# OpenMatchmaking/microservice-matchmaking

Hardware: AMD Instinct MI355X
Metric: matched players/sec over 1M-player pool (higher is better)
Workload: dtype int32

## Files before the change

### microservice_matchmaking_amd/csrc/mm_engine.hip

```cpp
#include <hip/hip_runtime.h>

#include <stdint.h>
#include <stdio.h>
#include <stdlib.h>
#include <string.h>
#include <time.h>

#include <dlfcn.h>

#include <algorithm>
#include <mutex>
#include <cmath>
#include <new>
#include <vector>

#include "../../include/mm_engine.h"
#include "../../include/mm_wait.h"
#include <mm_gfx950.h>


#define MM_NO_SLOT 0xFFFFFFFFu
#define MM_ST_FREE 0
#define MM_ST_LIVE 1
#define MM_ST_CANCELLED 2
// ... 774 lines not shown
    for (uint32_t k = 0; k < A.L; ++k) dst[k] = src[k];
    pk[(size_t)A.total * A.L + i] = __float_as_uint(out_score[(size_t)g * A.out_rec_stride + j]);
    pk[(size_t)A.total * (A.L + 1u) + i] = out_pass[(size_t)g * A.out_rec_stride + j];
}
__global__ __launch_bounds__(256) void k_wait_matched(PackArgs A, const uint32_t* __restrict__ out_slots,
                                                      const uint32_t* __restrict__ stamp, uint32_t capacity, uint32_t now,
                                                      uint32_t* __restrict__ wait)
{
    const uint32_t i = blockIdx.x * blockDim.x + threadIdx.x;
    if (i >= A.total * A.L) return;
    const uint32_t lobby = i / A.L;
    uint32_t g = 0;
    while (g + 1u < A.n_groups && lobby >= A.pre[g + 1u]) ++g;
    const uint32_t sl = out_slots[(size_t)g * A.out_slot_stride + (size_t)(i - A.pre[g] * A.L)];
    wait[i] = sl < capacity ? now - stamp[sl] : 0u;
}
#define MM_PACK_MAX 8192u

struct TailArgs {
    uint32_t pre[MM_MAX_GROUPS + 1];
    uint32_t from[MM_MAX_GROUPS], base[MM_MAX_GROUPS];
    uint32_t n_groups, L, total, out_slot_stride, out_rec_stride;
};
__global__ __launch_bounds__(256) void k_results_tail(TailArgs A, const uint32_t* __restrict__ out_slots,
                                                      const float* __restrict__ out_score, const uint32_t* __restrict__ out_pass,
                                                      uint32_t* __restrict__ h_slots, float* __restrict__ h_score, uint32_t* __restrict__ h_pass)
{
    const uint32_t i = blockIdx.x * blockDim.x + threadIdx.x;
    if (i >= A.total) return;
    uint32_t g = 0;
    while (g + 1u < A.n_groups && i >= A.pre[g + 1u]) ++g;
    const uint32_t j = A.from[g] + (i - A.pre[g]);
    const size_t at = (size_t)A.base[g] + j;
    const uint32_t* const src = out_slots + (size_t)g * A.out_slot_stride + (size_t)j * A.L;
    for (uint32_t k = 0; k < A.L; ++k) h_slots[at * A.L + k] = src[k];
    h_score[at] = out_score[(size_t)g * A.out_rec_stride + j];
    h_pass[at] = out_pass[(size_t)g * A.out_rec_stride + j];
}
#define MM_TAIL_MAX (1u << 20)

__global__ __launch_bounds__(256) void k_look(const uint32_t* __restrict__ src, uint32_t* __restrict__ dst_host, uint32_t nwords,
                                              uint32_t* seq_host, uint32_t seq)
{
    for (uint32_t i = threadIdx.x; i < nwords; i += blockDim.x) dst_host[i] = src[i];
    __threadfence_system();
    __syncthreads();
    if (threadIdx.x == 0) __hip_atomic_store(seq_host, seq, __ATOMIC_RELEASE, __HIP_MEMORY_SCOPE_SYSTEM);
}

#include "mm_pair.inc"
#include "mm_team.inc"

static __device__ __forceinline__ bool pair_chain_is_fast(const struct PairChain* pc, uint32_t g)
{
    return pc[g].fast != 0u;
// ... 76 lines not shown
    uint32_t* d_tk_chunkB;
    uint32_t* d_tk_fdone;
    uint32_t team_seq;
    uint32_t* d_tk_sqi;
    uint32_t tk_memb;
    uint32_t tk_chunk_stride;
    std::vector<uint32_t> tk_last_len;
    uint32_t dbg_last_w, dbg_last_c;
    ChainDev* h_chains;
    uint32_t* h_counters;
    std::vector<uint8_t> h_state;
    uint32_t next_slot;
    uint32_t cancel_pending;
    std::vector<uint32_t> r_released;
    uint32_t* h_rslots;
    float* h_rscore;
    uint32_t* h_rpass;
    uint32_t r_n, r_L;
    hipStream_t copy_stream;
    hipEvent_t ev_copy;
    bool ev_copy_pending;
    uint32_t r_base[MM_MAX_GROUPS], r_cnt[MM_MAX_GROUPS], r_pre[MM_MAX_GROUPS + 1];
    uint32_t r_sent[MM_MAX_GROUPS];
    uint32_t r_marked[MM_MAX_GROUPS];
    bool r_based;
    bool poisoned;
    uint32_t ticks_seen;
    bool clock_on;
    uint32_t clock_now;
    uint32_t* d_stamp;
    uint32_t* d_wt_rows;
    uint32_t wt_max_chunks;
    uint32_t* d_wt_out;
    WaitGroupDev* d_wt_stats;
    uint32_t* d_wt_matched;
    std::vector<uint32_t> x_slot, x_group, x_age;
    std::vector<uint32_t> x_new;
    std::vector<int32_t> x_rating;
    std::vector<uint32_t> x_cons, x_stamp;
    uint32_t* d_mv_cols;
    uint8_t* d_mv_group;
    uint32_t* h_mwait;
    uint32_t mw_n;
    uint32_t* d_loc_tag;
    uint32_t* d_loc_rows;
    uint32_t loc_max_chunks;
// ... 772 lines not shown
        if (live.empty()) return MM_OK;
        MMTRY(ensure_staging(e, live.size()));
        const uint32_t k = (uint32_t)live.size();
        HIPCHK(e, hipMemcpyAsync(e->d_in_slot, live.data(), k * sizeof(uint32_t), hipMemcpyHostToDevice, e->stream));
        hipLaunchKernelGGL(k_cancel, dim3((k + 255) / 256), dim3(256), 0, e->stream, k, e->d_in_slot, e->d_state);
        HIPCHK(e, hipGetLastError());
        HIPCHK(e, hipStreamSynchronize(e->stream));
        e->cancel_pending += k;
        return MM_OK;
    });
}

#ifndef MM_RESULTS_MIN_PAIR
#define MM_RESULTS_MIN_PAIR 16384u
#endif
#ifndef MM_RESULTS_MIN_TEAM
#define MM_RESULTS_MIN_TEAM 4096u
#endif
static void results_set_bases(mm_engine* e, const uint32_t* before, uint32_t L)
{
    uint32_t run = 0;
    for (uint32_t g = 0; g < e->cfg.n_groups; ++g) {
        e->r_base[g] = run;
        run += before[g] / L + 1u;
    }
    e->r_based = true;
}

static void results_mark(mm_engine* e, uint32_t g, uint32_t to, uint32_t L)
{
    const uint32_t from = e->r_marked[g];
    if (to <= from) return;
    const uint32_t* const sl = e->h_rslots + (size_t)(e->r_base[g] + from) * L;
    for (size_t i = 0, n = (size_t)(to - from) * L; i < n; ++i) e->h_state[sl[i]] = MM_ST_FREE;
    e->r_marked[g] = to;
}

static int results_absorb(mm_engine* e, uint32_t L)
{
    if (!e->ev_copy_pending) return MM_OK;
    HIPCHK(e, hipEventSynchronize(e->ev_copy));
    e->ev_copy_pending = false;
    for (uint32_t g = 0; g < e->cfg.n_groups; ++g) results_mark(e, g, e->r_sent[g], L);
    return MM_OK;
}

static int results_send(mm_engine* e, const uint32_t* n_out, uint32_t L, uint32_t min_new, bool* on_main = nullptr)
{
    uint32_t fresh = 0;
    for (uint32_t g = 0; g < e->cfg.n_groups; ++g) fresh += n_out[g] > e->r_sent[g] ? n_out[g] - e->r_sent[g] : 0u;
    if (on_main) *on_main = false;
    if (fresh < min_new) return MM_OK;
    MMTRY(results_absorb(e, L));
    if (on_main != nullptr && fresh <= MM_TAIL_MAX && e->tn.results_tail) {
        TailArgs A;
        memset(&A, 0, sizeof(A));
        A.n_groups = e->cfg.n_groups; A.L = L; A.out_slot_stride = e->out_slot_stride; A.out_rec_stride = e->out_rec_stride;
        for (uint32_t g = 0; g < e->cfg.n_groups; ++g) {
            const uint32_t a = e->r_sent[g], b = n_out[g] > a ? n_out[g] : a;
            A.from[g] = a; A.base[g] = e->r_base[g]; A.pre[g + 1u] = A.pre[g] + (b - a);
            e->r_sent[g] = b;
        }
        A.total = A.pre[e->cfg.n_groups];
        if (A.total) {
            hipLaunchKernelGGL(k_results_tail, dim3((A.total + 255u) / 256u), dim3(256), 0, e->stream, A, e->d_out_slots, e->d_out_score,
                               e->d_out_pass, e->h_rslots, e->h_rscore, e->h_rpass);
            HIPCHK(e, hipGetLastError());
        }
        *on_main = true;
        return MM_OK;
    }
    const bool main_st = on_main != nullptr && fresh <= 8192u;
    hipStream_t const st = main_st ? e->stream : e->copy_stream;
    for (uint32_t g = 0; g < e->cfg.n_groups; ++g) {
        const uint32_t a = e->r_sent[g], b = n_out[g];
        if (b <= a) continue;
        const size_t at = (size_t)e->r_base[g] + a;
        HIPCHK(e, hipMemcpyAsync(&e->h_rslots[at * L], e->d_out_slots + (size_t)g * e->out_slot_stride + (size_t)a * L,
                                 (size_t)(b - a) * L * sizeof(uint32_t), hipMemcpyDeviceToHost, st));
        HIPCHK(e, hipMemcpyAsync(&e->h_rscore[at], e->d_out_score + (size_t)g * e->out_rec_stride + a, (size_t)(b - a) * sizeof(float),
                                 hipMemcpyDeviceToHost, st));
        HIPCHK(e, hipMemcpyAsync(&e->h_rpass[at], e->d_out_pass + (size_t)g * e->out_rec_stride + a, (size_t)(b - a) * sizeof(uint32_t),
                                 hipMemcpyDeviceToHost, st));
        e->r_sent[g] = b;
    }
    if (main_st) { *on_main = true; return MM_OK; }
    HIPCHK(e, hipEventRecord(e->ev_copy, e->copy_stream));
    e->ev_copy_pending = true;
    return MM_OK;
// ... 148 lines not shown
    {
        uint32_t seg = 256u, stage = NXI_STAGE;
        while (seg < NXI_SEG && (unsigned long long)bound > 8192ull * seg) seg <<= 1;
        if (e->tn.pair_nxseg) seg = e->tn.pair_nxseg;
        if (e->tn.pair_nxstage) stage = e->tn.pair_nxstage;
        if (stage < seg + 64u) stage = seg + 64u;
        if (stage > NXI_STAGE) stage = NXI_STAGE;
        const bool timing = (cfg.flags & MM_CFG_TIMING) != 0;
        if (timing) HIPCHK(e, hipEventRecord(e->ev_nx[0], e->stream));
        hipLaunchKernelGGL(kp_nx_init, dim3((bound + seg - 1u) / seg + 1u, G), dim3(NXI_THREADS), 0, e->stream, P, seg, stage);
        if (timing) { HIPCHK(e, hipEventRecord(e->ev_nx[1], e->stream)); e->ev_nx_set = true; }
    }
    HIPCHK(e, hipGetLastError());
    uint32_t tail_no[MM_MAX_GROUPS];
    bool tail_send = false;
    memset(e->ps_hand, 0, sizeof(e->ps_hand));
    if (bound >= PL_MAX) {
        uint32_t tiles = (bound + PK_T - 1u) / PK_T + 1u;
        if (tiles > e->pk_max_tiles) tiles = e->pk_max_tiles;
        bool after_persist = false;
        uint32_t last_tp = 0;
        uint32_t idle_looks = 0;
        unsigned long long last_progress = ~0ull;
        for (uint32_t guard = 0;; ++guard) {
            if (idle_looks > 64u) return MM_ERR_INTERNAL;
            MMTRY(look_launch(e, e->d_pchains, e->h_pchains, G * sizeof(PairChain)));
            MMTRY(look_wait(e));
            ++e->ps.host_looks;
            if (e->tn.debug && guard >= 200u && guard % 200u == 0u) {
                fprintf(stderr, "[mm-pair] look %u: cool-down %u, persist %d, last tile length %u;", guard, e->pair_pcool, (int)kp_rounds_on(e), last_tp);
                for (uint32_t g = 0; g < G; ++g) {
                    const PairChain& pc = e->h_pchains[g];
                    if (pc.fast) fprintf(stderr, " g%u[stage %u m %u qlen %u passes %u compact %u pfail 0x%x]", g, pc.stage, pc.m, pc.qlen, pc.passes, pc.want_compact, pc.pfail);
                }
                fprintf(stderr, "\n");
            }
            {
                unsigned long long progress = 0;
                for (uint32_t g = 0; g < G; ++g) {
                    const PairChain& pc = e->h_pchains[g];
                    if (pc.fast) progress += (unsigned long long)pc.passes + ((unsigned long long)pc.m << 32) + (pc.stage == PS_TILED ? 1u : 0u) + pc.want_compact;
                }
                idle_looks = progress == last_progress ? idle_looks + 1u : 0u;
                last_progress = progress;
            }
            bool tiled = false, compact = false;
// ... 25 lines not shown
                uint32_t bf[MM_MAX_GROUPS];
                for (uint32_t g = 0; g < G; ++g) { bf[g] = e->h_pchains[g].before; sent_no[g] = e->h_pchains[g].fast ? e->h_pchains[g].n_out : 0u; }
                if (!e->r_based) results_set_bases(e, bf, M.L);
            }
            after_persist = false;
            for (uint32_t g = 0; g < G; ++g) {
                const PairChain& pc = e->h_pchains[g];
                if (!pc.fast) continue;
                if (pc.ppass > e->ps.pair_rounds_passes) e->ps.pair_rounds_passes = pc.ppass;
                if (pc.rounds > e->ps.pair_tiled_passes) e->ps.pair_tiled_passes = pc.rounds;
            }
            for (uint32_t g = 0; g < G; ++g) {
                const PairChain& pc = e->h_pchains[g];
                e->ps_hand[0][g] = pc.fast ? pc.passes : 0u;
                e->ps_hand[1][g] = pc.fast ? pc.n_out : 0u;
                e->ps_hand[2][g] = pc.fast ? pc.ppass : 0u;
                e->ps_hand[3][g] = pc.fast ? pc.ptm[15] : 0u;
            }
            if (!tiled) {
                if (guard) { for (uint32_t g = 0; g < G; ++g) tail_no[g] = sent_no[g]; tail_send = true; }
                break;
            }
            bool want_fit = false;
            uint32_t yield_q = 0, yield_g = 0;
            if (kp_rounds_on(e) && !e->pair_pcool && !compact && !e->tn.pair_tile_fixed) {
                uint32_t gl = 0;
                for (uint32_t g = 1; g < G; ++g)
                    if (P.bm[g] > P.bm[gl]) gl = g;
                const PairChain& pc = e->h_pchains[gl];
                if (P.bm[gl]) {
                    uint32_t capq = e->tn.pair_ptiles * PK_TMAX;
                    for (uint32_t tlen = PK_TMAX; tlen >= PK_TMAX / 4u && pc.m <= e->tn.pair_ptiles * tlen; tlen >>= 1) capq = e->tn.pair_ptiles * (tlen >> 1);
                    if (pc.m <= e->tn.pair_ptiles * (PK_TMAX / 4u)) capq = PL_MAX - 1u;
                    if (pc.qlen <= capq && pc.m > capq && capq >= PL_MAX) {
                        hipLaunchKernelGGL(kp_ask_compact, dim3(G), dim3(64), 0, e->stream, P, 1u << gl);
                        compact = true;
                    } else {
                        if (pc.m > e->tn.pair_ptiles * PK_TMAX) want_fit = true;
                        yield_q = capq;
                        yield_g = gl;
                    }
                }
            }
            uint32_t tp = PK_TMAX;
            bool persist = kp_rounds_on(e) && !compact && (longest + PK_TMAX - 1u) / PK_TMAX <= e->tn.pair_ptiles;
            if (persist && e->pair_pcool) { --e->pair_pcool; persist = false; e->ps.degraded = 1; }
            if (!kp_rounds_on(e) && !compact && (longest + PK_TMAX - 1u) / PK_TMAX <= e->tn.pair_ptiles) e->ps.degraded = 1;
            const uint32_t cap_p = e->tn.pair_ptiles < e->tn.pair_tiles_max ? e->tn.pair_ptiles : e->tn.pair_tiles_max;
            const uint32_t tiles_max = kp_rounds_on(e) ? cap_p : e->tn.pair_tiles_max;
            if (!e->tn.pair_tile_fixed)
                for (uint32_t cand = PK_TMAX / 4u; cand < PK_TMAX; cand <<= 1)
                    if ((longest + cand - 1u) / cand <= tiles_max) { tp = cand; break; }
            if (last_tp && tp > last_tp && !compact) {
                hipLaunchKernelGGL(kp_ask_compact, dim3(G), dim3(64), 0, e->stream, P, 0xFFFFFFFFu);
                compact = true;
                last_tp = 0;
            }
            tiles = (longest + tp - 1u) / tp;
#define TILE_LAUNCH(KERNEL, GRID, BLOCK, ...)                                                                              \
    do {                                                                                                                   \
        if (tp == PK_TMAX) hipLaunchKernelGGL(KERNEL<PK_TMAX>, GRID, BLOCK, 0, e->stream, __VA_ARGS__);                    \
// ... 27 lines not shown
                    if (slots) {
                        P.grp = 0;
                        const uint32_t K = e->tn.pair_pbatch, slice = MM_PERSIST_SLICE ? MM_PERSIST_SLICE : K + 1u;
                        for (uint32_t it = 0; it <= K; it += slice)
                            TILE_LAUNCH(kp_rounds, dim3(8u * slots), dim3(PT_THREADS), P, it, it + slice < K + 1u ? it + slice : K + 1u, K);
                        ++e->ps.pair_rounds_launches;
                        after_persist = true;
                        COMPACT_LAUNCH();
                        HIPCHK(e, hipGetLastError());
                        MMTRY(results_absorb(e, M.L));
                        MMTRY(results_send(e, sent_no, M.L, e->tn.results_early ? MM_RESULTS_MIN_PAIR : 0xFFFFFFFFu));
                        continue;
                    }
                    P.xslots = 0;
                }
                if (e->tn.pair_xcd) {
                    const uint32_t slots = pair_xcd_map(P, tof, G);
                    if (slots) rgrid = dim3(8u * slots);
                }
                uint32_t r = e->round_ctr;
                TILE_LAUNCH(kp_round, rgrid, dim3(PT_THREADS), P, r, 1u);
                ++r;
                if (P.grp) TILE_LAUNCH(kp_group, dim3(ngr, G), dim3(1024), P, r);
                for (uint32_t b = 0; b < (want_fit && e->tn.pair_batch > 12u ? 12u : e->tn.pair_batch); ++b) {
                    TILE_LAUNCH(kp_round, rgrid, dim3(PT_THREADS), P, r, 0u);
                    ++e->ps.pair_round_launches;
                    ++r;
                    if (P.grp) TILE_LAUNCH(kp_group, dim3(ngr, G), dim3(1024), P, r);
                }
                TILE_LAUNCH(kp_round_commit, dim3(tiles, G), dim3(256), P, r);
                hipLaunchKernelGGL(kp_round_stage, dim3(G), dim3(64), 0, e->stream, P, r);
                COMPACT_LAUNCH();
                e->round_ctr = r;
            }
#undef COMPACT_LAUNCH
#undef TILE_LAUNCH
            HIPCHK(e, hipGetLastError());
            MMTRY(results_absorb(e, M.L));
            MMTRY(results_send(e, sent_no, M.L, e->tn.results_early ? MM_RESULTS_MIN_PAIR : 0xFFFFFFFFu));
        }
    }
    hipLaunchKernelGGL(kp_late, dim3(G), dim3(PL_THREADS), 0, e->stream, P);
    hipLaunchKernelGGL(kp_finish, dim3(G), dim3(1024), 0, e->stream, P);
    HIPCHK(e, hipGetLastError());
    if (tail_send) {
        MMTRY(results_absorb(e, M.L));
        MMTRY(results_send(e, tail_no, M.L, e->tn.results_early ? MM_RESULTS_MIN_PAIR : 0xFFFFFFFFu));
// ... 411 lines not shown
    const bool use_pair = M.team_size == 1u && M.teams == 2u && !e->tn.force_generic;
    if (use_pair) {
        RoctxRange rr("mm_tick/pair walk");
        e->ps.paths |= MM_PATH_PAIR;
        MMTRY(pair_walk(e, mode, M, purge));
    }
    bool team_any = false;
    if (!use_pair && !e->tn.force_generic && e->live_upper >= TT_MIN) {
        RoctxRange rr("mm_tick/team walk");
        MMTRY(team_walk(e, mode, M, purge, &team_any));
        if (team_any) e->ps.paths |= MM_PATH_TEAM;
    }
    if (!e->ps.paths) e->ps.paths = MM_PATH_GENERIC;
    WalkParams P;
    walk_params_common(P, e, mode, purge);
    P.out_cap = (cfg.capacity + MM_MAX_LOBBY) / M.L + 1u;
    P.max_passes = 0x7FFFFFFFu;
    P.M = M;
    P.pskip = use_pair ? e->d_pchains : NULL;
    P.tskip = team_any ? e->d_tchains : NULL;
    hipLaunchKernelGGL(k_walk, dim3(G), dim3(WK_THREADS), 0, e->stream, P);
    HIPCHK(e, hipGetLastError());
    if (timing) HIPCHK(e, hipEventRecord(e->ev[2], e->stream));
    HIPCHK(e, hipMemcpyAsync(e->h_chains, e->d_chains, e->n_chains * sizeof(ChainDev), hipMemcpyDeviceToHost, e->stream));
    HIPCHK(e, hipMemcpyAsync(e->h_counters, e->d_counters, sizeof(uint32_t), hipMemcpyDeviceToHost, e->stream));
    if (use_pair) HIPCHK(e, hipMemcpyAsync(e->h_pchains, e->d_pchains, G * sizeof(PairChain), hipMemcpyDeviceToHost, e->stream));
    HIPCHK(e, hipStreamSynchronize(e->stream));
    const double t_copy0 = host_now_ms();
    if (use_pair && e->tn.debug) MMTRY(report_pair(e));

    uint32_t total = 0, after = 0, before = 0, pmax = 0, errf = 0;
    unsigned long long pairs = 0, scanned = 0;
    for (uint32_t g = 0; g < G; ++g) {
        const ChainDev& c = e->h_chains[mode * G + g];
        total += c.n_out;
        after += c.len + c.lobby.n;
        before += c.before;
        pairs += c.pairs;
        scanned += c.scanned;
        errf |= c.err;
        if (c.passes > pmax) pmax = c.passes;
    }
    if (errf) return MM_ERR_INTERNAL;
    if (e->tn.fail_tick && ++e->ticks_seen == e->tn.fail_tick) return MM_ERR_INTERNAL;
    if ((size_t)total * M.L > (size_t)cfg.capacity + (size_t)MM_MAX_LOBBY * G) return MM_ERR_INTERNAL;
    RoctxRange rr_res("mm_tick/match list");
    bool tail_on_main = false;
    {
        uint32_t bf[MM_MAX_GROUPS], no[MM_MAX_GROUPS];
        for (uint32_t g = 0; g < G; ++g) {
            const ChainDev& c = e->h_chains[mode * G + g];
            bf[g] = c.n_out * M.L;
            no[g] = c.n_out;
            if (e->r_based && (c.n_out < e->r_sent[g] || (unsigned long long)c.n_out * M.L > (unsigned long long)c.before + M.L))
                return MM_ERR_INTERNAL;
        }
        if (!e->r_based && total > 0u && total <= MM_PACK_MAX) {
            const PackArgs A = pack_args(e, mode, M.L, total);
            for (uint32_t g = 0; g < G; ++g) { e->r_base[g] = A.pre[g]; e->r_sent[g] = no[g]; }
            e->r_based = true;
            hipLaunchKernelGGL(k_pack_results, dim3((total + 255u) / 256u), dim3(256), 0, e->stream, A, e->d_out_slots, e->d_out_score,
                               e->d_out_pass, e->d_pack);
            HIPCHK(e, hipGetLastError());
            HIPCHK(e, hipMemcpyAsync(e->h_rslots, e->d_pack, (size_t)total * M.L * sizeof(uint32_t), hipMemcpyDeviceToHost, e->stream));
            HIPCHK(e, hipMemcpyAsync(e->h_rscore, e->d_pack + (size_t)total * M.L, (size_t)total * sizeof(float), hipMemcpyDeviceToHost, e->stream));
            HIPCHK(e, hipMemcpyAsync(e->h_rpass, e->d_pack + (size_t)total * (M.L + 1u), (size_t)total * sizeof(uint32_t), hipMemcpyDeviceToHost, e->stream));
            tail_on_main = true;
        } else {
            if (!e->r_based) results_set_bases(e, bf, M.L);
            MMTRY(results_send(e, no, M.L, 1u, &tail_on_main));
        }
    }
    const uint32_t nrel = e->h_counters[0];
    e->r_released.resize(nrel);
    if (nrel)
        HIPCHK(e, hipMemcpyAsync(e->r_released.data(), e->d_released, nrel * sizeof(uint32_t), hipMemcpyDeviceToHost, e->stream));
    if (e->clock_on && total > 0u) {
        const PackArgs A = pack_args(e, mode, M.L, total);
        const uint32_t words = total * M.L;
        hipLaunchKernelGGL(k_wait_matched, dim3((words + 255u) / 256u), dim3(256), 0, e->stream, A, e->d_out_slots, e->d_stamp,
                           cfg.capacity, e->clock_now, e->d_wt_matched);
        HIPCHK(e, hipGetLastError());
        HIPCHK(e, hipMemcpyAsync(e->h_mwait, e->d_wt_matched, (size_t)words * sizeof(uint32_t), hipMemcpyDeviceToHost, e->stream));
    }
    {
        MMTRY(results_absorb(e, M.L));
    }
    e->r_pre[0] = 0;
    for (uint32_t g = 0; g < G; ++g) {
        e->tk_last_len[mode * G + g] = e->h_chains[mode * G + g].len + e->h_chains[mode * G + g].lobby.n;
        e->r_cnt[g] = e->h_chains[mode * G + g].n_out;
        e->r_pre[g + 1u] = e->r_pre[g] + e->r_cnt[g];
    }
    HIPCHK(e, hipStreamSynchronize(e->stream));
    if (tail_on_main)
        for (uint32_t g = 0; g < G; ++g) results_mark(e, g, e->r_sent[g], M.L);
    for (uint32_t i = 0; i < nrel; ++i) e->h_state[e->r_released[i]] = MM_ST_FREE;
    e->cancel_pending = e->cancel_pending >= nrel ? e->cancel_pending - nrel : 0;
    {
        const unsigned long long gone = (unsigned long long)total * M.L + nrel;
        e->live_upper = e->live_upper >= gone ? e->live_upper - gone : 0;
    }
    e->r_n = total;
    e->mw_n = e->clock_on ? total : 0u;
    if (n_matches) *n_matches = total;
    if (e->ps.paths & MM_PATH_PAIR) path_stats_pair(e, mode);
    e->ps.crit_team_group = 0xFFFFFFFFu;
    if (e->ps.paths & MM_PATH_TEAM) path_stats_team(e);
    if (stats) {
        memset(stats, 0, sizeof(*stats));
        stats->pool_before = before;
        stats->pool_after = after;
        stats->matches = total;
        stats->players_matched = total * M.L;
        stats->passes_max = pmax;
        stats->chains = G;
        stats->pairs = pairs;
// ... 954 lines not shown
```

### microservice_matchmaking_amd/csrc/mm_pair.inc

```

#define PK_NO 0xFFFFFFFFu
#define PK_ABORT 0xFFFFFFFEu

#define NX_INV 0u
#define NX_NONE 0xFFFFu
#define NX_FAR 0xFFFEu

#ifndef PK_T
#define PK_T 8192u
#endif
enum : uint32_t { PK_TMAX = PK_T };
#undef PK_T
static constexpr uint32_t PK_T = PK_TMAX;
#ifndef PK_TILES_MAX
#define PK_TILES_MAX 40u
#endif
#define PK_XSEG 4u
#ifndef PK_GS
#define PK_GS 8u
#endif
#ifndef PK_GROUP_MIN
#define PK_GROUP_MIN 64u
#endif
#ifndef PL_MAX
// ... 1793 lines not shown
#undef EMIT_STORE
#undef SEAT_PATCH
}

#define PF_TIMEOUT 1u
#define PF_XCD 2u
#define PF_INJECT 3u
#define PF_YIELD 4u

template <uint32_t TP>
struct RoundsRes {
    alignas(16) uint32_t key[2 * TP + 64];
    alignas(16) uint16_t nx[TP];
    alignas(16) uint16_t g[TP + 8];
    alignas(16) uint32_t pc[TP + 64];
    alignas(16) uint32_t bits[2 * TP / 32 + 4];
    uint32_t cnt[16];
    uint16_t nw[TP / 32 + 2];
    uint16_t path[TP / 2 + 72];
    RoundState S, N;
    uint32_t my[8];
    uint32_t ctl[4];
    uint32_t tm[16];
};

static __device__ __forceinline__ uint32_t w_scan_fit_x(const uint32_t* key, const uint32_t* bits, uint32_t akey, uint32_t from, uint32_t m,
                                                        uint32_t w, int lane)
{
    uint32_t klo, krng;
    pk_bounds(akey, w, klo, krng);
    for (uint32_t p = from; p < m; p += 256u) {
        uint32_t bw[4], kv[4];
#pragma unroll
        for (uint32_t u = 0; u < 4u; ++u) {
            const uint32_t c = p + 64u * u + (uint32_t)lane;
            bw[u] = c < m ? xld(bits + (c >> 5)) : 0u;
            kv[u] = c < m ? key[c] : 0xFFFFFFFFu;
        }
#pragma unroll
        for (uint32_t u = 0; u < 4u; ++u) {
            const uint32_t c = p + 64u * u + (uint32_t)lane;
            const unsigned long long b = __ballot(((bw[u] >> (c & 31u)) & 1u) != 0u && pk_in(kv[u], klo, krng));
            if (b) return p + 64u * u + (uint32_t)__ffsll(b) - 1u;
        }
    }
    return PK_NO;
// ... 29 lines not shown
                t = ((sg >> 8) & 0xFFu) + sl * (sg >> 16);
                found = true;
            }
            if (!found) sl -= c;
        }
        if (!found) return;
    }
    PairChain* const pc = P.pchains + g;
    const uint32_t m = P.bm[g], buf = P.bbuf[g];
    if (m == 0u || t >= (m + PK_T - 1u) / PK_T) return;
    const int tid_o = threadIdx.x;
    const uint32_t w = P.window, ntiles = (m + PK_T - 1u) / PK_T;
    const uint32_t c = P.mode * P.n_groups + g;
    const size_t qo = (size_t)c * P.capacity, po = (size_t)g * P.pstride;
    const uint32_t base = t * PK_T;
    const uint32_t tl = dev_min_u32(PK_T, m - base);
    const uint32_t hl = dev_min_u32(2u * PK_T, m - base);
    const uint32_t* const key = P.key[buf] + po;
    const uint32_t* const oidx = P.oidx[buf] + po;
    uint16_t* const gnx = P.nx16[buf] + po + base;
    uint32_t* const bits_com = P.bits[buf] + (size_t)g * P.bits_stride;
    const uint32_t own_words = (tl + 31u) >> 5, hwords = (hl + 31u) >> 5;
    unsigned long long* const bar = P.pbar + g;
    long long tq = clock64();
#define TMARK(K_) do { if (tmr) { const long long now = clock64(); L.tm[K_] += (uint32_t)(now - tq); tq = now; } } while (0)

    if (it_begin == 0u) {
        const int tid = tid_o;
        MM_RESIDENT_FRESH(L);
        if (tid == 0) {
            RoundState S;
            S.live = 1; S.done = 0; S.want_compact = 0; S.rounds = pc->rounds;
            S.qlen = pc->qlen; S.passes = pc->passes; S.n_out = pc->n_out; S.has_anchor = pc->has_anchor;
            S.a_key = pc->a_key; S.a_slot = pc->a_slot; S.a_cons = pc->a_cons; S.a_team = pc->a_team;
            S.a_rating = pc->a_rating; S.pairs = pc->pairs; S.scanned = pc->scanned;
            S.pos0 = pc->pos0; S.changed0 = pc->changed0; S.extra0 = pc->extra0; S.a_oi = PK_NO;
            L.S = S;
            L.N = S;
            L.ctl[0] = 0; L.ctl[1] = 0; L.ctl[2] = 0;
            for (int k = 0; k < 16; ++k) L.tm[k] = 0;
        }
        for (uint32_t i = tid; i < 2u * PK_T / 32u + 4u; i += PT_THREADS) s_bits[i] = i < hwords ? bits_com[(base >> 5) + i] : 0u;
        copy_words_x4((uint32_t*)s_nx, (const uint32_t*)gnx, (tl + 1u) >> 1, tid, PT_THREADS);
        if (tid < 8) s_g[PK_T + tid] = (uint16_t)PK_T;
        if (tid == 0) { s_cnt[1] = 0; s_cnt[2] = 0; s_cnt[3] = 0; s_cnt[4] = 0; }
        if ((uint32_t)tid < RP_MAXLONG) s_pc[RP_MAXLONG + tid] = PK_NO;
        __syncthreads();
        prep_stage_keys<PK_T>(s_key, s_bits, key + base, hl, tid);
        __syncthreads();
    } else if (L.ctl[0]) return;

    uint32_t stop = 0;
    bool ended = false;
    uint32_t tst = 0;
    long long dw0 = 0;
    uint32_t dwork = 0, dn = 0;
    for (uint32_t it = it_begin; it < it_end; ++it) {
        int tid_l = tid_o;
        TW_LAUNDER(tid_l);
        const int tid = tid_l, lane = tid & 63, wave = tid >> 6;
        const bool tmr = t == 1u && tid == 0;
        const uint32_t cpar = it & 1u, npar = cpar ^ 1u;
        const uint32_t* const bits_src = P.bitsp[cpar] + (size_t)g * P.bits_stride;
        uint32_t* const bits_dst = P.bitsp[npar] + (size_t)g * P.bits_stride;
        uint32_t em_off = PK_NO, em_ia = 0, em_iq = 0, em_score = 0, hd_off = PK_NO, hd_iq = 0, hd_score = 0;
        uint32_t em_sa = 0, em_sq = 0, hd_sq = 0, hd_sa = 0, hd_team = 0, em_pass = 0;
        bool em_loaded = false;
#define EMIT_LOAD() do { if (!em_loaded) { em_loaded = true;                                                   \
        if (em_off != PK_NO) { em_sa = P.q_slot[qo + em_ia]; em_sq = P.q_slot[qo + em_iq]; }                  \
        if (hd_off != PK_NO) hd_sq = P.q_slot[qo + hd_iq]; } } while (0)
#define EMIT_STORE() do { EMIT_LOAD();                                                                         \
        uint32_t* const eos = P.out_slots + (size_t)g * P.out_slot_stride;                                    \
        if (em_off != PK_NO) {                                                                                \
            eos[2u * em_off] = em_sa; eos[2u * em_off + 1u] = em_sq;                                          \
            P.out_score[(size_t)g * P.out_rec_stride + em_off] = (float)(int32_t)em_score;                    \
            P.out_pass[(size_t)g * P.out_rec_stride + em_off] = em_pass; }                                    \
        if (hd_off != PK_NO) {                                                                                \
            eos[2u * hd_off + hd_team] = hd_sa; eos[2u * hd_off + (1u - hd_team)] = hd_sq;                    \
            P.out_score[(size_t)g * P.out_rec_stride + hd_off] = (float)(int32_t)hd_score;                    \
            P.out_pass[(size_t)g * P.out_rec_stride + hd_off] = em_pass; }                                    \
        em_off = PK_NO; hd_off = PK_NO; } while (0)

        if (it > 0u) {
            if (tid == 0) {
// ... 8 lines not shown
                    if ((wv & 0xFFFFFFFFull) >= need) break;
                    if (f == 0u && xld(P.pyield) != 0u) {
                        const unsigned long long nv = wv | ((unsigned long long)(PF_YIELD | (it << 8)) << 32);
                        if (atomicCAS(bar, wv, nv) == wv) { verdict = PF_YIELD | (it << 8); break; }
                        continue;
                    }
                    if (f == 0u && wall_clock64() - t0 > limit) {
                        const unsigned long long nv = wv | ((unsigned long long)(PF_TIMEOUT | (it << 8)) << 32);
                        if (atomicCAS(bar, wv, nv) == wv) { verdict = PF_TIMEOUT | (it << 8); break; }
                        continue;
                    }
                    __builtin_amdgcn_s_sleep(1);
                }
                if (!verdict && it == 1u) {
                    const uint32_t xm = xld(P.pxmask + g);
                    if (xm & (xm - 1u)) verdict = PF_XCD | (1u << 8);
                }
                L.ctl[1] = verdict;
            }
            __syncthreads();
            tw_sinv();
            if (L.ctl[1]) { stop = L.ctl[1]; break; }
            TMARK(0);
            if (tid == 0 && (P.tune & 0x10000u)) dw0 = clock64();
            const RoundState S = L.S;
            em_pass = S.passes;
            if (wave != 0) {
                for (uint32_t i = PK_T / 32u + (uint32_t)tid - 64u; i < hwords; i += PT_THREADS - 64u) {
                    const uint32_t nw_ = xld(bits_src + (base >> 5) + i);
                    uint32_t gone = s_bits[i] & ~nw_;
                    s_bits[i] = nw_;
                    while (gone) {
                        const uint32_t b = (uint32_t)__ffs((int)gone) - 1u;
                        gone &= gone - 1u;
                        s_key[(i << 5) + b] |= PK_DEAD;
                    }
                }
                if ((uint32_t)tid - 64u < RP_MAXLONG) s_pc[RP_MAXLONG + tid - 64] = PK_NO;
                __builtin_amdgcn_fence(__ATOMIC_RELEASE, "workgroup");
                wave_lockstep();
                if (lane == 0) atomicAdd(&s_cnt[4], 1u);
                while (lds_ld(&s_cnt[4]) < (uint32_t)(PT_THREADS / 64 - 1)) __builtin_amdgcn_s_sleep(1);
                __builtin_amdgcn_fence(__ATOMIC_ACQUIRE, "workgroup");
                if (it != K && !(P.tune & 0x4000u))
                    repair_sweep<PK_T>(s_key, s_nx, s_pc, &s_cnt[1], s_pc + 2u * RP_MAXLONG + (uint32_t)wave * RP_TODO, bits_src + (base >> 5),
                                       tl, hl, base + hl == m, w, lane, (uint32_t)wave - 1u, PT_THREADS / 64u - 1u, tst);
            }
// ... 196 lines not shown
                        em_score = sc;
                    } else {
                        os[2u * (my_off + i)] = P.q_slot[qo + oidx[base + a]];
                        os[2u * (my_off + i) + 1u] = P.q_slot[qo + oidx[qabs]];
                        P.out_score[(size_t)g * P.out_rec_stride + my_off + i] = (float)(int32_t)sc;
                        P.out_pass[(size_t)g * P.out_rec_stride + my_off + i] = em_pass;
                    }
                }
            }
            if (tid == 0) {
                if (n) {
                    const uint32_t a = s_path[n - 1u], o = s_nx[a];
                    const bool internal = o != NX_NONE && o != NX_FAR && a + o < tl;
                    if (internal && d != DISP_NONE) atomicOr(&pc->err, MM_ERRF_SEAT_INVARIANT);
                } else if (d != DISP_NONE) atomicOr(&pc->err, MM_ERRF_SEAT_INVARIANT);
                L.S = L.N;
                L.ctl[2] += 1u;
            }
            __syncthreads();
            TMARK(9);
        }
        struct { uint32_t live, has_anchor, a_key; } N;
        N.live = L.S.live; N.has_anchor = L.S.has_anchor; N.a_key = L.S.a_key;
        if (!N.live || it == K) { EMIT_STORE(); ended = true; break; }
        if (it > 0u && L.S.qlen <= P.pyq[g]) {
            if (t == 0u && tid == 0) __hip_atomic_store(P.pyield, 1u, __ATOMIC_RELAXED, __HIP_MEMORY_SCOPE_AGENT);
            EMIT_STORE(); ended = true; break;
        }

        for (uint32_t i = tid; i < own_words; i += PT_THREADS) bits_dst[(base >> 5) + i] = s_bits[i];
        if (tid == 0) { s_cnt[0] = PK_NO; s_cnt[4] = 0; }
        prep_repair<PK_T>(s_key, s_nx, s_pc, &s_cnt[1], bits_src + (base >> 5), tl, hl, base + hl == m, w, tid, tst,
                          tmr ? L.tm : nullptr);
        EMIT_LOAD();
        if (N.has_anchor) {
            uint32_t klo, krng;
            pk_bounds(N.a_key, w, klo, krng);
            uint32_t best = PK_NO;
            for (uint32_t i = tid; i < tl; i += PT_THREADS)
                if (best == PK_NO && pk_in(s_key[i], klo, krng)) best = i;
            const unsigned long long b = __ballot(best != PK_NO);
            if (b) {
                uint32_t v = best;
                for (int dd = 1; dd < 64; dd <<= 1) { const uint32_t o2 = (uint32_t)__shfl((int)v, lane ^ dd); v = o2 < v ? o2 : v; }
                if (lane == 0) atomicMin(&s_cnt[0], v);
            }
        }
        prep_tables<PK_T>(s_key, s_nx, s_bits, s_nw, s_pc, s_g, P.rec2[npar] + po + base, P.exa[npar] + po + base,
                          nullptr, tl, tid, tmr ? L.tm : nullptr);
        if (tmr) tq = clock64();
        if (tid == 0) P.headp[npar][(size_t)g * P.max_tiles + t] = s_cnt[0] == PK_NO ? PK_NO : base + s_cnt[0];
        {
            uint32_t acc = 0;
            const uint32_t* const rb = P.rec2[npar] + po + base;
            for (uint32_t i = (uint32_t)tid * 16u; i < tl; i += PT_THREADS * 16u) acc ^= xld(rb + i);
            for (uint32_t i = (uint32_t)tid * 16u; i < own_words; i += PT_THREADS * 16u) acc ^= xld(bits_dst + (base >> 5) + i);
            TW_SINK(acc);
        }
        tw_store_wait();
        __syncthreads();
        if (tid == 0) {
            unsigned long long add = 1ull;
            if (it == 0u) {
                const uint32_t o = atomicOr(P.pxmask + g, 1u << mm_xcc_id());
                TW_KEEP(o);
                tw_store_wait();
            }
            if (it > 0u && (P.tune & 0x10000u)) { dwork += (uint32_t)(clock64() - dw0); ++dn; }
            if (P.pinject && P.pinject == it && t == 1u) {
                for (;;) {
                    const unsigned long long o = xld64(bar);
                    if (o >> 32) { atomicAdd(bar, 1ull); break; }
                    if (atomicCAS(bar, o, (o + 1ull) | ((unsigned long long)(PF_INJECT | ((it + 1u) << 8)) << 32)) == o) break;
                }
            } else atomicAdd(bar, add);
        }
        EMIT_STORE();
        TMARK(4);
    }
#undef EMIT_LOAD
#undef EMIT_STORE
    if (!ended && !stop) return;

    const int tid = tid_o, lane = tid & 63;
    const bool tmr = t == 1u && tid == 0;
    __syncthreads();
    for (uint32_t i = tid; i < own_words; i += PT_THREADS) bits_com[(base >> 5) + i] = s_bits[i];
    for (uint32_t i = tid; i < tl; i += PT_THREADS)
        if (s_nx[i] == NX_PEND) s_nx[i] = (uint16_t)NX_INV;
    __syncthreads();
    {
        uint4* const nx4 = (uint4*)gnx;
        for (uint32_t i = tid; i < (tl + 7u) >> 3; i += PT_THREADS) nx4[i] = ((const uint4*)s_nx)[i];
    }
    if (tid == 0) L.ctl[0] = 1;
    if (t == 0 && tid == 0) {
        const RoundState S = L.S;
        pc->qlen = S.qlen; pc->passes = S.passes; pc->n_out = S.n_out; pc->has_anchor = S.has_anchor;
        pc->a_key = S.a_key; pc->a_team = S.a_team;
        if (S.has_anchor && S.a_oi != PK_NO) {
            pc->a_slot = P.q_slot[qo + S.a_oi]; pc->a_rating = P.q_rating[qo + S.a_oi]; pc->a_cons = P.q_cons[qo + S.a_oi];
        } else { pc->a_slot = S.a_slot; pc->a_rating = S.a_rating; pc->a_cons = S.a_cons; }
        pc->pairs = S.pairs; pc->scanned = S.scanned; pc->rounds = S.rounds;
        pc->want_compact = S.want_compact | ((!S.done && P.pyq[g] && S.qlen <= P.pyq[g]) ? 1u : 0u);
        pc->pos0 = S.pos0; pc->changed0 = S.changed0; pc->extra0 = S.extra0;
        if (S.done) pc->stage = PS_DONE;
        pc->pfail = stop;
        pc->ppass += L.ctl[2];
        pc->pxm = xld(P.pxmask + g);
    }
    if (tmr) {
        for (int k = 0; k < 16; ++k) if (L.tm[k]) atomicAdd(&pc->ptm[k], L.tm[k]);
        atomicAdd(&pc->ptm[5], L.ctl[2]);
    }
    if ((P.tune & 0x2000u) && lane == 0 && tst) atomicAdd(&pc->tested, (unsigned long long)tst);
    if ((P.tune & 0x10000u) && tid == 0 && dn) {
        uint32_t* const dg = (uint32_t*)(P.grec + (size_t)g * P.gstride + t);
        atomicAdd(dg + 0, dwork);
        atomicAdd(dg + 1, dn);
    }
#undef TMARK
}

template <uint32_t TP>
__global__ __launch_bounds__(1024) void kp_group(PairParams P, uint32_t r_next)
{
    constexpr uint32_t PK_T = TP;
    (void)PK_T;
    const uint32_t g = blockIdx.y, gr = blockIdx.x;
    const uint32_t m = P.bm[g];
    if (m == 0u) return;
    const uint32_t ntiles = (m + PK_T - 1u) / PK_T;
    if (gr * P.grp >= ntiles) return;
    const uint32_t cpar = r_next & 1u;
    if (!(P.pchains + g)->rs[cpar].live) return;
    const size_t po = (size_t)g * P.pstride;
    const uint32_t* const rec = P.rec2[cpar] + po;
    const uint32_t* const bits = P.bitsp[cpar] + (size_t)g * P.bits_stride;
    uint4* const out = P.grec + (size_t)g * P.gstride + (size_t)gr * PK_T;
    const uint32_t t0 = gr * P.grp, gend = t0 + P.grp;
    __shared__ uint32_t s_mark[PK_T / 32u];
    __shared__ uint32_t s_list[PK_T];
// ... 292 lines not shown
```

Before: 105.6 million.

## Launch results tail early, adapt fit batch, and trim pair-round register state

After the walk kernel, a results-tail copy kernel is now launched speculatively over each group's reserved room. It reads the device chain counts to skip rows that were never produced, so the host stream synchronize can be skipped when nothing else needs it. The fit-mode round batch is now estimated from observed queue shrinkage per pass instead of being fixed at 12. The pair kernel moves its timing and debug counters into shared state, flushes the per-iteration tested counter, and replaces the first-match min-reduction with a ballot/ffs scan that exits early. Together these aim to cut host syncs, excess round launches and register pressure, at the cost of extra copy threads over unused room and more complex control flow.

```diff
diff --git a/microservice_matchmaking_amd/csrc/mm_engine.hip b/microservice_matchmaking_amd/csrc/mm_engine.hip
--- a/microservice_matchmaking_amd/csrc/mm_engine.hip
+++ b/microservice_matchmaking_amd/csrc/mm_engine.hip
@@ -820,7 +820,7 @@
     uint32_t from[MM_MAX_GROUPS], base[MM_MAX_GROUPS];
     uint32_t n_groups, L, total, out_slot_stride, out_rec_stride;
 };
-__global__ __launch_bounds__(256) void k_results_tail(TailArgs A, const uint32_t* __restrict__ out_slots,
+__global__ __launch_bounds__(256) void k_results_tail(TailArgs A, const ChainDev* __restrict__ chains, const uint32_t* __restrict__ out_slots,
                                                       const float* __restrict__ out_score, const uint32_t* __restrict__ out_pass,
                                                       uint32_t* __restrict__ h_slots, float* __restrict__ h_score, uint32_t* __restrict__ h_pass)
 {
@@ -829,6 +829,7 @@
     uint32_t g = 0;
     while (g + 1u < A.n_groups && i >= A.pre[g + 1u]) ++g;
     const uint32_t j = A.from[g] + (i - A.pre[g]);
+    if (chains != nullptr && j >= chains[g].n_out) return;
     const size_t at = (size_t)A.base[g] + j;
     const uint32_t* const src = out_slots + (size_t)g * A.out_slot_stride + (size_t)j * A.L;
     for (uint32_t k = 0; k < A.L; ++k) h_slots[at * A.L + k] = src[k];
@@ -951,6 +952,7 @@
     bool ev_copy_pending;
     uint32_t r_base[MM_MAX_GROUPS], r_cnt[MM_MAX_GROUPS], r_pre[MM_MAX_GROUPS + 1];
     uint32_t r_sent[MM_MAX_GROUPS];
+    uint32_t r_room[MM_MAX_GROUPS];
     uint32_t r_marked[MM_MAX_GROUPS];
     bool r_based;
     bool poisoned;
@@ -1769,7 +1771,8 @@
     uint32_t run = 0;
     for (uint32_t g = 0; g < e->cfg.n_groups; ++g) {
         e->r_base[g] = run;
-        run += before[g] / L + 1u;
+        e->r_room[g] = before[g] / L + 1u;
+        run += e->r_room[g];
     }
     e->r_based = true;
 }
@@ -1810,8 +1813,8 @@
         }
         A.total = A.pre[e->cfg.n_groups];
         if (A.total) {
-            hipLaunchKernelGGL(k_results_tail, dim3((A.total + 255u) / 256u), dim3(256), 0, e->stream, A, e->d_out_slots, e->d_out_score,
-                               e->d_out_pass, e->h_rslots, e->h_rscore, e->h_rpass);
+            hipLaunchKernelGGL(k_results_tail, dim3((A.total + 255u) / 256u), dim3(256), 0, e->stream, A, (const ChainDev*)nullptr, e->d_out_slots,
+                               e->d_out_score, e->d_out_pass, e->h_rslots, e->h_rscore, e->h_rpass);
             HIPCHK(e, hipGetLastError());
         }
         *on_main = true;
@@ -2006,6 +2009,7 @@
         uint32_t last_tp = 0;
         uint32_t idle_looks = 0;
         unsigned long long last_progress = ~0ull;
+        uint32_t fit_g = 0xFFFFFFFFu, fit_qlen = 0, fit_passes = 0;
         for (uint32_t guard = 0;; ++guard) {
             if (idle_looks > 64u) return MM_ERR_INTERNAL;
             MMTRY(look_launch(e, e->d_pchains, e->h_pchains, G * sizeof(PairChain)));
@@ -2077,6 +2081,7 @@
                 break;
             }
             bool want_fit = false;
+            uint32_t fit_batch = e->tn.pair_batch > 12u ? 12u : e->tn.pair_batch;
             uint32_t yield_q = 0, yield_g = 0;
             if (kp_rounds_on(e) && !e->pair_pcool && !compact && !e->tn.pair_tile_fixed) {
                 uint32_t gl = 0;
@@ -2091,7 +2096,15 @@
                         hipLaunchKernelGGL(kp_ask_compact, dim3(G), dim3(64), 0, e->stream, P, 1u << gl);
                         compact = true;
                     } else {
-                        if (pc.m > e->tn.pair_ptiles * PK_TMAX) want_fit = true;
+                        if (pc.m > e->tn.pair_ptiles * PK_TMAX) {
+                            want_fit = true;
+                            if (fit_g == gl && pc.passes > fit_passes && pc.qlen < fit_qlen && pc.qlen > capq) {
+                                const unsigned long long need = pc.qlen - capq, dq = fit_qlen - pc.qlen, dp = pc.passes - fit_passes;
+                                const unsigned long long nb = (need * dp + dq - 1ull) / dq;
+                                fit_batch = nb < 1ull ? 1u : nb > (unsigned long long)e->tn.pair_batch ? e->tn.pair_batch : (uint32_t)nb;
+                            }
+                            fit_g = gl; fit_qlen = pc.qlen; fit_passes = pc.passes;
+                        }
                         yield_q = capq;
                         yield_g = gl;
                     }
@@ -2165,7 +2178,7 @@
                 TILE_LAUNCH(kp_round, rgrid, dim3(PT_THREADS), P, r, 1u);
                 ++r;
                 if (P.grp) TILE_LAUNCH(kp_group, dim3(ngr, G), dim3(1024), P, r);
-                for (uint32_t b = 0; b < (want_fit && e->tn.pair_batch > 12u ? 12u : e->tn.pair_batch); ++b) {
+                for (uint32_t b = 0, nb = want_fit ? fit_batch : e->tn.pair_batch; b < nb; ++b) {
                     TILE_LAUNCH(kp_round, rgrid, dim3(PT_THREADS), P, r, 0u);
                     ++e->ps.pair_round_launches;
                     ++r;
@@ -2623,6 +2636,29 @@
     hipLaunchKernelGGL(k_walk, dim3(G), dim3(WK_THREADS), 0, e->stream, P);
     HIPCHK(e, hipGetLastError());
     if (timing) HIPCHK(e, hipEventRecord(e->ev[2], e->stream));
+    bool tail_early = false;
+    if (e->r_based && e->tn.results_tail) {
+        TailArgs A;
+        memset(&A, 0, sizeof(A));
+        A.n_groups = G; A.L = M.L; A.out_slot_stride = e->out_slot_stride; A.out_rec_stride = e->out_rec_stride;
+        unsigned long long most = 0;
+        for (uint32_t g = 0; g < G; ++g) {
+            const uint32_t a = e->r_sent[g], room = e->r_room[g] > a ? e->r_room[g] - a : 0u;
+            A.from[g] = a; A.base[g] = e->r_base[g];
+            most += room;
+            A.pre[g + 1u] = (uint32_t)(most <= MM_TAIL_MAX ? most : MM_TAIL_MAX);
+        }
+        if (most <= MM_TAIL_MAX) {
+            A.total = (uint32_t)most;
+            if (A.total) {
+                hipLaunchKernelGGL(k_results_tail, dim3((A.total + 255u) / 256u), dim3(256), 0, e->stream, A,
+                                   (const ChainDev*)(e->d_chains + (size_t)mode * G), e->d_out_slots, e->d_out_score, e->d_out_pass,
+                                   e->h_rslots, e->h_rscore, e->h_rpass);
+                HIPCHK(e, hipGetLastError());
+            }
+            tail_early = true;
+        }
+    }
     HIPCHK(e, hipMemcpyAsync(e->h_chains, e->d_chains, e->n_chains * sizeof(ChainDev), hipMemcpyDeviceToHost, e->stream));
     HIPCHK(e, hipMemcpyAsync(e->h_counters, e->d_counters, sizeof(uint32_t), hipMemcpyDeviceToHost, e->stream));
     if (use_pair) HIPCHK(e, hipMemcpyAsync(e->h_pchains, e->d_pchains, G * sizeof(PairChain), hipMemcpyDeviceToHost, e->stream));
@@ -2655,8 +2691,12 @@
             no[g] = c.n_out;
             if (e->r_based && (c.n_out < e->r_sent[g] || (unsigned long long)c.n_out * M.L > (unsigned long long)c.before + M.L))
                 return MM_ERR_INTERNAL;
-        }
-        if (!e->r_based && total > 0u && total <= MM_PACK_MAX) {
+            if (tail_early && c.n_out > e->r_room[g]) return MM_ERR_INTERNAL;
+        }
+        if (tail_early) {
+            for (uint32_t g = 0; g < G; ++g) e->r_sent[g] = no[g];
+            tail_on_main = true;
+        } else if (!e->r_based && total > 0u && total <= MM_PACK_MAX) {
             const PackArgs A = pack_args(e, mode, M.L, total);
             for (uint32_t g = 0; g < G; ++g) { e->r_base[g] = A.pre[g]; e->r_sent[g] = no[g]; }
             e->r_based = true;
@@ -2693,7 +2733,7 @@
         e->r_cnt[g] = e->h_chains[mode * G + g].n_out;
         e->r_pre[g + 1u] = e->r_pre[g] + e->r_cnt[g];
     }
-    HIPCHK(e, hipStreamSynchronize(e->stream));
+    if (!tail_early || nrel || (e->clock_on && total > 0u)) HIPCHK(e, hipStreamSynchronize(e->stream));
     if (tail_on_main)
         for (uint32_t g = 0; g < G; ++g) results_mark(e, g, e->r_sent[g], M.L);
     for (uint32_t i = 0; i < nrel; ++i) e->h_state[e->r_released[i]] = MM_ST_FREE;
diff --git a/microservice_matchmaking_amd/csrc/mm_pair.inc b/microservice_matchmaking_amd/csrc/mm_pair.inc
--- a/microservice_matchmaking_amd/csrc/mm_pair.inc
+++ b/microservice_matchmaking_amd/csrc/mm_pair.inc
@@ -1839,6 +1839,9 @@
     uint32_t my[8];
     uint32_t ctl[4];
     uint32_t tm[16];
+    long long tq;
+    long long dw0;
+    uint32_t dwork, dn;
 };
 
 static __device__ __forceinline__ uint32_t w_scan_fit_x(const uint32_t* key, const uint32_t* bits, uint32_t akey, uint32_t from, uint32_t m,
@@ -1914,8 +1917,7 @@
     uint32_t* const bits_com = P.bits[buf] + (size_t)g * P.bits_stride;
     const uint32_t own_words = (tl + 31u) >> 5, hwords = (hl + 31u) >> 5;
     unsigned long long* const bar = P.pbar + g;
-    long long tq = clock64();
-#define TMARK(K_) do { if (tmr) { const long long now = clock64(); L.tm[K_] += (uint32_t)(now - tq); tq = now; } } while (0)
+#define TMARK(K_) do { if (tmr) { const long long now = clock64(); L.tm[K_] += (uint32_t)(now - L.tq); L.tq = now; } } while (0)
 
     if (it_begin == 0u) {
         const int tid = tid_o;
@@ -1931,6 +1933,7 @@
             L.N = S;
             L.ctl[0] = 0; L.ctl[1] = 0; L.ctl[2] = 0;
             for (int k = 0; k < 16; ++k) L.tm[k] = 0;
+            L.dw0 = 0; L.dwork = 0; L.dn = 0;
         }
         for (uint32_t i = tid; i < 2u * PK_T / 32u + 4u; i += PT_THREADS) s_bits[i] = i < hwords ? bits_com[(base >> 5) + i] : 0u;
         copy_words_x4((uint32_t*)s_nx, (const uint32_t*)gnx, (tl + 1u) >> 1, tid, PT_THREADS);
@@ -1941,17 +1944,17 @@
         prep_stage_keys<PK_T>(s_key, s_bits, key + base, hl, tid);
         __syncthreads();
     } else if (L.ctl[0]) return;
+    if (t == 1u && tid_o == 0) L.tq = clock64();
 
     uint32_t stop = 0;
     bool ended = false;
-    uint32_t tst = 0;
-    long long dw0 = 0;
-    uint32_t dwork = 0, dn = 0;
     for (uint32_t it = it_begin; it < it_end; ++it) {
         int tid_l = tid_o;
         TW_LAUNDER(tid_l);
         const int tid = tid_l, lane = tid & 63, wave = tid >> 6;
         const bool tmr = t == 1u && tid == 0;
+        uint32_t tst = 0;
+#define TST_FLUSH() do { if ((P.tune & 0x2000u) && lane == 0 && tst) atomicAdd(&pc->tested, (unsigned long long)tst); } while (0)
         const uint32_t cpar = it & 1u, npar = cpar ^ 1u;
         const uint32_t* const bits_src = P.bitsp[cpar] + (size_t)g * P.bits_stride;
         uint32_t* const bits_dst = P.bitsp[npar] + (size_t)g * P.bits_stride;
@@ -2006,7 +2009,7 @@
             tw_sinv();
             if (L.ctl[1]) { stop = L.ctl[1]; break; }
             TMARK(0);
-            if (tid == 0 && (P.tune & 0x10000u)) dw0 = clock64();
+            if (tid == 0 && (P.tune & 0x10000u)) L.dw0 = clock64();
             const RoundState S = L.S;
             em_pass = S.passes;
             if (wave != 0) {
@@ -2249,10 +2252,10 @@
         }
         struct { uint32_t live, has_anchor, a_key; } N;
         N.live = L.S.live; N.has_anchor = L.S.has_anchor; N.a_key = L.S.a_key;
-        if (!N.live || it == K) { EMIT_STORE(); ended = true; break; }
+        if (!N.live || it == K) { EMIT_STORE(); TST_FLUSH(); ended = true; break; }
         if (it > 0u && L.S.qlen <= P.pyq[g]) {
             if (t == 0u && tid == 0) __hip_atomic_store(P.pyield, 1u, __ATOMIC_RELAXED, __HIP_MEMORY_SCOPE_AGENT);
-            EMIT_STORE(); ended = true; break;
+            EMIT_STORE(); TST_FLUSH(); ended = true; break;
         }
 
         for (uint32_t i = tid; i < own_words; i += PT_THREADS) bits_dst[(base >> 5) + i] = s_bits[i];
@@ -2264,18 +2267,16 @@
             uint32_t klo, krng;
             pk_bounds(N.a_key, w, klo, krng);
             uint32_t best = PK_NO;
-            for (uint32_t i = tid; i < tl; i += PT_THREADS)
-                if (best == PK_NO && pk_in(s_key[i], klo, krng)) best = i;
-            const unsigned long long b = __ballot(best != PK_NO);
-            if (b) {
-                uint32_t v = best;
-                for (int dd = 1; dd < 64; dd <<= 1) { const uint32_t o2 = (uint32_t)__shfl((int)v, lane ^ dd); v = o2 < v ? o2 : v; }
-                if (lane == 0) atomicMin(&s_cnt[0], v);
-            }
+            for (uint32_t i0 = (uint32_t)wave * 64u; i0 < tl && best == PK_NO; i0 += PT_THREADS) {
+                const uint32_t i = i0 + (uint32_t)lane;
+                const unsigned long long b = __ballot(i < tl && pk_in(s_key[i], klo, krng));
+                if (b) best = i0 + (uint32_t)__ffsll(b) - 1u;
+            }
+            if (best != PK_NO && lane == 0) atomicMin(&s_cnt[0], best);
         }
         prep_tables<PK_T>(s_key, s_nx, s_bits, s_nw, s_pc, s_g, P.rec2[npar] + po + base, P.exa[npar] + po + base,
                           nullptr, tl, tid, tmr ? L.tm : nullptr);
-        if (tmr) tq = clock64();
+        if (tmr) L.tq = clock64();
         if (tid == 0) P.headp[npar][(size_t)g * P.max_tiles + t] = s_cnt[0] == PK_NO ? PK_NO : base + s_cnt[0];
         {
             uint32_t acc = 0;
@@ -2293,7 +2294,7 @@
                 TW_KEEP(o);
                 tw_store_wait();
             }
-            if (it > 0u && (P.tune & 0x10000u)) { dwork += (uint32_t)(clock64() - dw0); ++dn; }
+            if (it > 0u && (P.tune & 0x10000u)) { L.dwork += (uint32_t)(clock64() - L.dw0); L.dn += 1u; }
             if (P.pinject && P.pinject == it && t == 1u) {
                 for (;;) {
                     const unsigned long long o = xld64(bar);
@@ -2303,13 +2304,15 @@
             } else atomicAdd(bar, add);
         }
         EMIT_STORE();
-        TMARK(4);
-    }
+ TMARK(4);
+        TST_FLUSH();
+    }
+#undef TST_FLUSH
 #undef EMIT_LOAD
 #undef EMIT_STORE
     if (!ended && !stop) return;
 
-    const int tid = tid_o, lane = tid & 63;
+    const int tid = tid_o;
     const bool tmr = t == 1u && tid == 0;
     __syncthreads();
     for (uint32_t i = tid; i < own_words; i += PT_THREADS) bits_com[(base >> 5) + i] = s_bits[i];
@@ -2340,11 +2343,10 @@
         for (int k = 0; k < 16; ++k) if (L.tm[k]) atomicAdd(&pc->ptm[k], L.tm[k]);
         atomicAdd(&pc->ptm[5], L.ctl[2]);
     }
-    if ((P.tune & 0x2000u) && lane == 0 && tst) atomicAdd(&pc->tested, (unsigned long long)tst);
-    if ((P.tune & 0x10000u) && tid == 0 && dn) {
+    if ((P.tune & 0x10000u) && tid == 0 && L.dn) {
         uint32_t* const dg = (uint32_t*)(P.grec + (size_t)g * P.gstride + t);
-        atomicAdd(dg + 0, dwork);
-        atomicAdd(dg + 1, dn);
+        atomicAdd(dg + 0, L.dwork);
+        atomicAdd(dg + 1, L.dn);
     }
 #undef TMARK
 }
```

Result: no change. 105.9 million, median of 4 (+0.3%).
